# Tavish9/freegaussian

Hardware: AMD Instinct MI355X
Metric: Mpixels/s fwd+bwd @ 1M Gaussians 1080p (higher is better)
Workload: dtype f32; 1 GPU; north-star cfg4: 1000000 Gaussians, 1920x1080, SH degree 3, 1 view per rank per step, view = (rank + step) mod 8 around the 8-view ring, fwd+bwd, RGB, absgrad; layout=uniform, N=1000000, P=2073600, parallelism=view-dp1

## Files before the change

### freegaussian_amd/csrc/raster.hip

```cpp
#include "fg_common.h"

#include <stdlib.h>
#include <string.h>

#include <type_traits>

#include "jobs_build.h"

namespace {
using namespace fgjobs;

constexpr int TILE = 16;

__host__ __device__ constexpr int rec_vec4(int C) { return (6 + C + 3) / 4; }

__device__ __forceinline__ int tile_of_block(int b, int n, int tile_w, int tile_h, int mode) {
  const int xcd = b & 7, k = b >> 3;
  const int only = ((mode >> 8) & 15) - 1, kmod = mode >> 12;
  mode &= 255;
  if (only >= 0 && xcd != only) return -1;
  if (kmod > 1 && k % kmod != 0) return -1;
  if (mode == 0) {
    const int row = (k / tile_w) * 8 + xcd;
    return row < tile_h ? row * tile_w + (k % tile_w) : -1;
// ... 741 lines not shown
                                                     const int32_t* __restrict__ tile_offsets,
                                                     const int32_t* __restrict__ flatten_ids, float* __restrict__ render,
                                                     float* __restrict__ alphas, int32_t* __restrict__ last_ids,
                                                     const Composite& comp, float4* __restrict__ ckpt,
                                                     uint32_t* __restrict__ live_words,
                                                     const int32_t* __restrict__ slot_tab, long long* __restrict__ walk_out,
                                                     int seg_fine) {
  constexpr int C = 3, NV = rec_vec4(C);
  constexpr float MAY_STOP = FG_T_STOP * 1.00001f;
  const int tile_y = tile / tile_w, tile_x = tile - tile_y * tile_w;
  const int n_tiles = tile_w * ((height + TILE - 1) / TILE);
  const int start = tile_offsets[tile], end = tile_offsets[tile + 1];
  const int slot0 = ckpt ? seg_slot_base(slot_tab, start, tile) : -1;
  if (slot0 < 0 || end - start <= FG_WIDE_PREFIX) return;
  float4* const slots = ckpt + seg_slots_offset4(n_tiles, width, height);
  const int lane = fg::lane_id(), w = __builtin_amdgcn_readfirstlane(threadIdx.x >> 6);
  FwdShared<3, 64>& st = sh.stage[w];
  const uint64_t lt_mask = (lane == 0) ? 0ull : (~0ull >> (64 - lane));
  const int col = lane & 15, row = 4 * strip + (lane >> 4);
  const int ix = tile_x * TILE + col, iy = tile_y * TILE + row;
  const bool inside = ix < width && iy < height;
  const size_t pix = (size_t)min(iy, height - 1) * width + min(ix, width - 1);
  const float px = (float)ix + 0.5f;
  const StripBounds sb = strip_bounds((float)(tile_x * TILE), (float)(tile_y * TILE));
  const float pyb = (float)(tile_y * TILE + (lane >> 4)) + 0.5f;
  const float strip_off = (float)(4 * strip);
  const uint64_t full = __ballot(true);
  {
    const float4 v = slots[seg_slot_index(slot0, start, start) * FG_SEG_SLOT4 + row * TILE + col];
    if (!__any(v.x > 0.f)) return;
    if (w == 0) {
      sh.base[lane] = make_float4(fabsf(v.x), v.y, v.z, v.w);
      sh.base_last[lane] = last_ids[pix];
      sh.base_w[lane] = -1;
      sh.base_fin[lane] = !(v.x > 0.f);
    }
  }
  int cnt = 0;
  int ev_mine = 0, sc_mine = 0;
  uint32_t vlo = 0, vhi = 0;
  auto walk = [&](int batch, float& T, float (&acc)[C], int& last, uint64_t& done, auto bits) {
    for (int n0 = 0; n0 < cnt; n0 += 8) {
      if (done == full) break;
      const int n1 = min(n0 + 8, cnt);
      unsigned next_v = st.list[0][n0];
      for (int n = n0; n < n1; ++n) {
        const unsigned packed = __builtin_amdgcn_readfirstlane(next_v);
        next_v = st.list[0][min(n + 1, 63)];
        const int j = packed & 255u;
        Splat s;
        float f[C];
        read_record<C>(st.rec[j], s, f);
        const float dx = s.x - px, dy_base = s.y - pyb;
        const SigmaTerms sg = sigma_terms_prescaled(s.a, s.b, s.c, dx);
        const float dy = dy_base - strip_off;
        const float e2 = neg_sigma_log2e(sg, dy);
        const float alpha = fminf(FG_ALPHA_MAX, s.o * __builtin_amdgcn_exp2f(e2));
        const uint64_t valid = lanes_ule(e2, 0.f) & lanes_oge(alpha, FG_ALPHA_SKIP) & ~done;
        if (valid == 0ull) continue;
        if constexpr (decltype(bits)::value) {
          if (j < 32) vlo |= (uint32_t)lane_select(valid, 1 << j, 0);
          else vhi |= (uint32_t)lane_select(valid, 1 << (j - 32), 0);
        }
        const float next_T = T * (1.f - alpha);
        const uint64_t stop = valid & lanes_ole(next_T, FG_T_STOP);
        const uint64_t take = valid & ~stop;
        const float vis = lane_select0(take, alpha * T);
#pragma unroll
        for (int c = 0; c < C; ++c) acc[c] += f[c] * vis;
        last = lane_select(take, batch + j, last);
        T = lane_select(take, next_T, T);
        done |= stop;
      }
    }
  };

  float4 v_next[NV];
  {
    const int idx = start + FG_WIDE_PREFIX + 64 * w + lane;
    if (idx < end) {
      const float4* rec = splats + (size_t)flatten_ids[idx] * (FG_SPLAT_FLOATS / 4);
#pragma unroll
      for (int q = 0; q < NV; ++q) v_next[q] = rec[q];
    }
  }
  for (int r0 = start + FG_WIDE_PREFIX; r0 < end; r0 += 64 * NWV) {
    __syncthreads();
    const uint64_t done0 = __ballot(sh.base_fin[lane] != 0);
    if (done0 == full) break;
    const int batch = r0 + 64 * w;
    const int idx_next = batch + 64 * NWV + lane;
    const int gid_next = idx_next < end ? flatten_ids[idx_next] : 0;
    float T = 1.f, acc[C] = {0.f, 0.f, 0.f};
    int last = -1;
    uint64_t done = done0;
    cnt = 0;
    vlo = vhi = 0;
    if (batch < end) {
      const int idx = batch + lane;
      unsigned mask = 0;
      if (idx < end) {
        float4 v[NV];
#pragma unroll
        for (int q = 0; q < NV; ++q) v[q] = v_next[q];
        mask = strip_mask(v[0].x, v[0].y, v[0].z, v[0].w, v[1].x, v[1].y, sb);
        v[0].w *= 0.5f * FG_NEG_LOG2E;
        v[1].x *= FG_NEG_LOG2E;
        v[1].y *= 0.5f * FG_NEG_LOG2E;
#pragma unroll
        for (int q = 0; q < NV; ++q) st.rec[lane][q] = v[q];
      }
      const bool rel = (mask >> strip) & 1u;
      const uint64_t bal = __ballot(rel);
      if (rel) st.list[0][__popcll(bal & lt_mask)] = (uint16_t)(lane | (mask << 8));
      cnt = __popcll(bal);
      ev_mine += cnt;
      sc_mine += min(64, end - batch);
      __builtin_amdgcn_fence(__ATOMIC_RELEASE, "wavefront");
      __builtin_amdgcn_wave_barrier();
      __builtin_amdgcn_fence(__ATOMIC_ACQUIRE, "wavefront");
      walk(batch, T, acc, last, done, std::true_type{});
    }
    if (idx_next < end) {
      const float4* rec = splats + (size_t)gid_next * (FG_SPLAT_FLOATS / 4);
#pragma unroll
      for (int q = 0; q < NV; ++q) v_next[q] = rec[q];
    }
    {
      const bool stopped = ((done & ~done0) >> lane) & 1ull;
      sh.part[w][lane] = make_float4(stopped ? -1.f : T, acc[0], acc[1], acc[2]);
      sh.part_last[w][lane] = last;
    }
    if (lane < 2) sh.live_or[w][lane] = 0u;
    float t_in = 1.f, c_in[C] = {0.f, 0.f, 0.f};
    int l_in = start - 1, bw = -1;
    bool fin = false;
    float4 ck = make_float4(1.f, 0.f, 0.f, 0.f);
    float4 mp = make_float4(1.f, 0.f, 0.f, 0.f);
    __syncthreads();
    for (;;) {
      bw = sh.base_w[lane];
      fin = sh.base_fin[lane] != 0;
      l_in = sh.base_last[lane];
      {
        const float4 b = sh.base[lane];
        t_in = b.x; c_in[0] = b.y; c_in[1] = b.z; c_in[2] = b.w;
      }
      bool earlier = false;
      for (int q0 = 0; q0 < w; q0 += 5) {
        float4 pq[5];
        int plq[5];
#pragma unroll
        for (int u = 0; u < 5; ++u) {
          const int qq = min(q0 + u, NWV - 1);
          pq[u] = sh.part[qq][lane];
          plq[u] = sh.part_last[qq][lane];
        }
#pragma unroll
        for (int u = 0; u < 5; ++u) {
          const float4 p = pq[u];
          const int q = q0 + u;
          const bool use = q < w && q > bw && !fin && !earlier;
          const bool ms = use && (p.x < 0.f || t_in * p.x <= MAY_STOP);
          earlier = earlier || ms;
          if (use && !ms) {
            c_in[0] = fmaf(t_in, p.y, c_in[0]);
            c_in[1] = fmaf(t_in, p.z, c_in[1]);
            c_in[2] = fmaf(t_in, p.w, c_in[2]);
            t_in *= p.x;
            l_in = plq[u] >= 0 ? plq[u] : l_in;
          }
        }
      }
      mp = sh.part[w][lane];
      const bool reached = w > bw && !fin && !earlier;
      if (reached) ck = make_float4(t_in, c_in[0], c_in[1], c_in[2]);
      const bool mine = reached && (mp.x < 0.f || t_in * mp.x <= MAY_STOP);
      const uint64_t active = __ballot(mine);
      if (!__syncthreads_or(active != 0ull)) break;
      bool went_on = false;
      if (active != 0ull) {
        uint64_t d2 = ~active;
        walk(batch, t_in, c_in, l_in, d2, std::false_type{});
        if (mine) {
          sh.base[lane] = make_float4(t_in, c_in[0], c_in[1], c_in[2]);
          sh.base_last[lane] = l_in;
          sh.base_w[lane] = w;
          sh.base_fin[lane] = (int)((d2 >> lane) & 1ull);
          went_on = !((d2 >> lane) & 1ull);
        }
      }
      if (!__syncthreads_or(went_on)) {
        fin = sh.base_fin[lane] != 0;
        if (fin) l_in = sh.base_last[lane];
        if (fin) bw = sh.base_w[lane];
        break;
      }
    }
    if (batch > start && batch < end && seg_starts_at(batch - start, seg_fine))
      slots[seg_slot_index(slot0, start, batch, seg_fine) * FG_SEG_SLOT4 + row * TILE + col] = ck;
    if (live_words && batch < end) {
      const int rel_last = fin ? l_in - batch : 63;
      const uint32_t klo = rel_last < 0 ? 0u : (rel_last >= 31 ? ~0u : (2u << rel_last) - 1u);
      const uint32_t khi = rel_last < 32 ? 0u : (rel_last >= 63 ? ~0u : (2u << (rel_last - 32)) - 1u);
      if (vlo & klo) atomicOr(&sh.live_or[w][0], vlo & klo);
      if (vhi & khi) atomicOr(&sh.live_or[w][1], vhi & khi);
      __builtin_amdgcn_fence(__ATOMIC_RELEASE, "wavefront");
      __builtin_amdgcn_wave_barrier();
      __builtin_amdgcn_fence(__ATOMIC_ACQUIRE, "wavefront");
      const uint32_t word = sh.live_or[w][lane >> 5];
      if (batch + lane < end) reinterpret_cast<uint8_t*>(live_words + (batch + lane))[strip] = (uint8_t)((word >> (lane & 31)) & 1u);
    }
    if (w == NWV - 1) {
      if (!fin) {
        if (w > bw) {
          c_in[0] = fmaf(t_in, mp.y, c_in[0]);
          c_in[1] = fmaf(t_in, mp.z, c_in[1]);
          c_in[2] = fmaf(t_in, mp.w, c_in[2]);
          t_in *= mp.x;
          const int pl = sh.part_last[w][lane];
          l_in = pl >= 0 ? pl : l_in;
        }
        sh.base[lane] = make_float4(t_in, c_in[0], c_in[1], c_in[2]);
        sh.base_last[lane] = l_in;
      }
      sh.base_w[lane] = -1;
    }
  }
  __syncthreads();
  if (w != 0) return;
  const float4 b = sh.base[lane];
  const int last = sh.base_last[lane];
  float accf[C] = {b.y, b.z, b.w};
  {
    const int m = fg::wave_max_i32(last);
    if (lane == 0) reinterpret_cast<int32_t*>(ckpt)[4 * tile + strip] = m;
    const long long reach = (long long)(m - start + 1) * ev_mine / max(sc_mine, 1);
    if (walk_out && reach > FG_WALK_REPORT && lane == 0)
      __hip_atomic_store(walk_out, reach, __ATOMIC_RELAXED, __HIP_MEMORY_SCOPE_SYSTEM);
  }
  if (inside) {
    const float alpha_out = 1.f - b.x;
    reinterpret_cast<float*>(ckpt + seg_plane_offset4(n_tiles))[pix] = b.x;
    if (comp.background || comp.n_clamp > 0) {
      const float om = 1.f - alpha_out;
      unsigned blocked = 0;
#pragma unroll
      for (int c = 0; c < C; ++c) {
        float v = accf[c];
        if (comp.background) v += om * comp.background[c];
        if (c < comp.n_clamp) {
          if (v < 0.f || v > 1.f) blocked |= 1u << c;
          v = fminf(fmaxf(v, 0.f), 1.f);
        }
        accf[c] = v;
      }
      if (comp.n_clamp > 0) comp.clamp_mask[pix] = (uint8_t)blocked;
    }
#pragma unroll
    for (int c = 0; c < C; ++c) render[pix * C + c] = accf[c];
    alphas[pix] = alpha_out;
    last_ids[pix] = last;
  }
}

static_assert(sizeof(WideShared<FG_WIDE_WAVES>) <= 160 * 1024 / 2, "a wide job's stages: two workgroups per CU of gfx950's 160 KB LDS");
#if defined(__HIP_DEVICE_COMPILE__) && !defined(__gfx950__)
#error "libfgraster's kernels are written for gfx950 (MI355X): 160 KB of LDS per CU, wave64; build with --offload-arch=gfx950"
#endif
__global__ void __launch_bounds__(64 * FG_WIDE_WAVES)
raster_fwd_wide_kernel(int width, int height, int tile_w, int32_t* __restrict__ open_list,
                       const float4* __restrict__ splats, const int32_t* __restrict__ tile_offsets,
                       const int32_t* __restrict__ flatten_ids, float* __restrict__ render, float* __restrict__ alphas,
                       int32_t* __restrict__ last_ids, Composite comp, float4* __restrict__ ckpt,
                       uint32_t* __restrict__ live_words, const int32_t* __restrict__ slot_tab,
                       long long* __restrict__ walk_out, int seg_fine) {
  __shared__ WideShared<FG_WIDE_WAVES> sh;
  const int n_open = __builtin_amdgcn_readfirstlane(open_list[0]);
  for (int v = blockIdx.x; v < n_open; v += gridDim.x) {
    const int e = open_list[8 + v];
    FG_TL_BEGIN();
    raster_fwd_wide_body<FG_WIDE_WAVES>(sh, e >> 3, (e & 7) - 1, width, height, tile_w, splats, tile_offsets, flatten_ids,
                                        render, alphas, last_ids, comp, ckpt, live_words, slot_tab, walk_out, seg_fine);
    __syncthreads();
    FG_TL_END(1, e >> 3, (e & 7) - 1, 0, 3);
  }
  if (threadIdx.x == 0) {
    __threadfence();
    if (atomicAdd(&open_list[1], 1) == (int)gridDim.x - 1) {
      open_list[0] = 0;
      open_list[1] = 0;
    }
  }
}

template <int C, int NT>
struct BwdShared {
  float4 rec[NT][rec_vec4(C)];
  int32_t gid[NT];
  uint32_t mask[NT];
  alignas(16) float red[NT / 64][(8 + C) * fg::FG_RED_STRIDE];
  int32_t mx[NT / 64];
};

template <int C, int PPT, int NW, bool LIVE = false>
__device__ __forceinline__ void raster_bwd_body(BwdShared<C, 64 * NW>& sh, int tile, int wave_base, int width,
                                                int height, int tile_w, const float4* __restrict__ splats,
                                                const int32_t* __restrict__ tile_offsets,
                                                const int32_t* __restrict__ flatten_ids,
                                                const float* __restrict__ alphas,
                                                const int32_t* __restrict__ last_ids,
                                                const float* __restrict__ v_render,
                                                const float* __restrict__ v_alphas, float* __restrict__ v_splats,
                                                const Composite& comp, const Segments& seg = Segments{nullptr, nullptr, nullptr, 1, 0, 0},
                                                int part = 0, const uint32_t* __restrict__ live_words = nullptr) {
  constexpr int NT = 64 * NW;
  constexpr int RSTEP = TILE / PPT;
  constexpr int NV = rec_vec4(C);
  auto& lds = sh.rec;
  auto& lds_gid = sh.gid;
  auto& lds_mask = sh.mask;
  auto& lds_max = sh.mx;
  auto& lds_red = sh.red;
  const int tile_y = tile / tile_w, tile_x = tile - tile_y * tile_w;
  const int start = tile_offsets[tile], end = tile_offsets[tile + 1];
  if (end <= start) return;
  const int lane = fg::lane_id(), wl = NW == 1 ? 0 : __builtin_amdgcn_readfirstlane(threadIdx.x >> 6),
            wave = wave_base + wl;
  const int col = threadIdx.x & 15, row0 = 4 * wave_base + (threadIdx.x >> 4);
  const int ix = tile_x * TILE + col;
  const float px = (float)ix + 0.5f;
  const StripBounds sb = strip_bounds((float)(tile_x * TILE), (float)(tile_y * TILE));
  const unsigned my_strips = wave_strips<PPT>(wave);

  float T[PPT], rest[PPT], vr[PPT][C];
  const float pyb = (float)(tile_y * TILE + (int)(threadIdx.x >> 4) - 4 * wl) + 0.5f;
  int last[PPT];
  int my_max = start - 1;
  FG_TL_MARK(0);
  int lo = start, hi = end, bin_final = start - 1;
  int slot_last[PPT];
  bool from_ckpt = false;
  const float4* ck_slot = nullptr;
  bool share_job = false;
  if constexpr (C == 3 && NW == 1) share_job = seg.ckpt && seg.parts > 1;
  if (share_job) {
    const int4 tl = reinterpret_cast<const int4*>(seg.ckpt)[tile];
    const int tls[4] = {tl.x, tl.y, tl.z, tl.w};
#pragma unroll
    for (int k = 0; k < PPT; ++k) {
      slot_last[k] = __builtin_amdgcn_readfirstlane(tls[wave + k * (4 / PPT)]);
      bin_final = max(bin_final, slot_last[k]);
    }
    const int n_used = bin_final - start + 1;
    if (n_used <= 0) return;
    const int nseg = seg_count(n_used, seg.fine);
    const int c0 = part * nseg / seg.parts, c1 = (part + 1) * nseg / seg.parts;
    if (c0 == c1) return;
    lo = start + seg_bound(c0, seg.fine);
    hi = bin_final + 1;
    if (c1 < nseg) {
      hi = start + seg_bound(c1, seg.fine);
      from_ckpt = true;
      ck_slot = seg.ckpt + seg_slots_offset4(tile_w * ((height + TILE - 1) / TILE), width, height) +
                seg_slot_index(seg_slot_base(seg.slot_tab, start, tile), start, hi, seg.fine) * FG_SEG_SLOT4;
    }
  }
  FG_TL_MARK(1);
  struct Px {
    float alpha, va;
    int last;
    unsigned blocked;
    float v[C];
  } raw[PPT];
  float4 ckv[PPT];
  float cfv[PPT][3], tfe[PPT];
  const float* t_exact = nullptr;
  if constexpr (C == 3 && NW == 1) {
    if (from_ckpt)
      t_exact = reinterpret_cast<const float*>(seg.ckpt + seg_plane_offset4(tile_w * ((height + TILE - 1) / TILE)));
  }
  {
    const int ixc = min(ix, width - 1);
#pragma unroll
    for (int k = 0; k < PPT; ++k) {
      const int iyc = min(tile_y * TILE + row0 + k * RSTEP, height - 1);
      const size_t pix = (size_t)iyc * width + ixc;
      raw[k].alpha = alphas[pix];
      raw[k].last = last_ids[pix];
#pragma unroll
      for (int c = 0; c < C; ++c) raw[k].v[c] = v_render[pix * C + c];
    }
    if (v_alphas) {
#pragma unroll
      for (int k = 0; k < PPT; ++k)
        raw[k].va = v_alphas[(size_t)min(tile_y * TILE + row0 + k * RSTEP, height - 1) * width + ixc];
    } else {
#pragma unroll
      for (int k = 0; k < PPT; ++k) raw[k].va = 0.f;
    }
    if (comp.n_clamp > 0) {
#pragma unroll
      for (int k = 0; k < PPT; ++k)
        raw[k].blocked = comp.clamp_mask[(size_t)min(tile_y * TILE + row0 + k * RSTEP, height - 1) * width + ixc];
    } else {
#pragma unroll
      for (int k = 0; k < PPT; ++k) raw[k].blocked = 0u;
    }
#pragma unroll
    for (int k = 0; k < PPT; ++k) {
      ckv[k] = make_float4(1.f, 0.f, 0.f, 0.f);
      cfv[k][0] = cfv[k][1] = cfv[k][2] = 0.f;
      tfe[k] = 1.f;
    }
    if constexpr (C == 3 && NW == 1) {
      if (from_ckpt) {
#pragma unroll
        for (int k = 0; k < PPT; ++k) {
          const int iyc = min(tile_y * TILE + row0 + k * RSTEP, height - 1);
          const size_t pix = (size_t)iyc * width + ixc;
          ckv[k] = ck_slot[(row0 + k * RSTEP) * TILE + col];
          tfe[k] = t_exact[pix];
#pragma unroll
          for (int c = 0; c < 3; ++c) cfv[k][c] = seg.render_raw[pix * 3 + c];
        }
      }
    }
  }
#pragma unroll
  for (int k = 0; k < PPT; ++k) {
    const int iy = tile_y * TILE + row0 + k * RSTEP;
    const bool inside = ix < width && iy < height;
    const float alpha_f = inside ? raw[k].alpha : 0.f;
    T[k] = 1.f - alpha_f;
    last[k] = inside ? raw[k].last : start - 1;
    float va = inside ? raw[k].va : 0.f;
    const unsigned blocked = inside ? raw[k].blocked : 0u;
#pragma unroll
    for (int c = 0; c < C; ++c) {
      float v = inside ? raw[k].v[c] : 0.f;
      if ((blocked >> c) & 1u) v = 0.f;
      if (comp.background) va -= v * comp.background[c];
      vr[k][c] = v;
    }
    rest[k] = T[k] * va;
    if constexpr (C == 3 && NW == 1) {
      if (from_ckpt) {
        const float prefix[3] = {ckv[k].y, ckv[k].z, ckv[k].w};
        float sfx = 0.f;
#pragma unroll
        for (int c = 0; c < 3; ++c) {
          float f = cfv[k][c];
          if (comp.background) f -= (1.f - alpha_f) * comp.background[c];
          sfx += vr[k][c] * (f - prefix[c]);
        }
        const bool resume = last[k] >= hi;
        const float rho = T[k] * __builtin_amdgcn_rcpf(fmaxf(tfe[k], 1e-30f));
        T[k] = resume ? ckv[k].x * rho : T[k];
        rest[k] -= resume ? sfx * rho : 0.f;
      }
    }
    my_max = max(my_max, last[k]);
  }
  FG_TL_MARK(2);
  if (!share_job) {
    bin_final = __builtin_amdgcn_readfirstlane(fg::wave_max_i32(my_max));
    if (NW > 1) {
      if (lane == 0) lds_max[wl] = bin_final;
      __syncthreads();
#pragma unroll
      for (int w = 0; w < NW; ++w) bin_final = max(bin_final, lds_max[w]);
    }
    if (bin_final - start + 1 <= 0) return;
    hi = bin_final + 1;
    if constexpr (LIVE) {
#pragma unroll
      for (int k = 0; k < PPT; ++k) slot_last[k] = __builtin_amdgcn_readfirstlane(fg::wave_max_i32(last[k]));
    }
  }
  const int n_used = bin_final - start + 1;
  (void)n_used;
  const int n_batches = (hi - lo + NT - 1) / NT;
  if (threadIdx.x == 0) { FG_STAT(5, n_used); FG_STAT(6, end - start); }
  uint32_t red_wr[(8 + C + 3) / 4];
#pragma unroll
  for (int i = 0; i < (8 + C + 3) / 4; ++i) red_wr[i] = fg::lds_opaque(&lds_red[wl][4 * i * fg::FG_RED_STRIDE + lane]);
  float g[16];
#pragma unroll
  for (int q = 0; q < 16; ++q) asm volatile("v_mov_b32 %0, 0" : "=v"(g[q]));

  for (int b = n_batches - 1; b >= 0; --b) {
    const int batch = __builtin_amdgcn_readfirstlane(lo + b * NT);
    __syncthreads();
    FG_TL_STAGE_BEGIN();
    const int tl = NW == 1 ? fresh_lane_id() : (int)threadIdx.x;
    const int idx = batch + tl;
    unsigned mask = 0;
    const int gid_early = (LIVE && idx < hi) ? flatten_ids[idx] : 0;
    if constexpr (LIVE) {
      if (idx < hi) {
        const uint32_t lw = live_words[idx];
#pragma unroll
        for (int k = 0; k < PPT; ++k) {
          const int s4 = wave + k * (4 / PPT);
          if (((lw >> (8 * s4)) & 1u) && idx <= slot_last[k]) mask |= 1u << s4;
        }
      }
    }
    if (LIVE ? mask != 0u : idx < hi) {
      const int gid = LIVE ? gid_early : flatten_ids[idx];
      lds_gid[tl] = gid;
      const float4* rec = splats + (size_t)gid * (FG_SPLAT_FLOATS / 4);
      float4 v[NV];
#pragma unroll
      for (int q = 0; q < NV; ++q) v[q] = rec[q];
      if constexpr (!LIVE) mask = strip_mask(v[0].x, v[0].y, v[0].z, v[0].w, v[1].x, v[1].y, sb);
      if constexpr (C == 3) {
        v[2].y = v[0].w * (0.5f * FG_NEG_LOG2E);
        v[2].z = v[1].x * FG_NEG_LOG2E;
        v[2].w = v[1].y * (0.5f * FG_NEG_LOG2E);
      }
#pragma unroll
      for (int q = 0; q < NV; ++q) lds[tl][q] = v[q];
    }
    lds_mask[tl] = mask;
    __syncthreads();
    FG_TL_STAGE_END();
    for (int i = NT / 64 - 1; i >= 0; --i) {
      uint64_t todo = __ballot((lds_mask[64 * i + lane] & my_strips) != 0u);
      while (todo != 0ull) {
        const int bit = 63 - __builtin_clzll(todo);
        todo &= ~(1ull << bit);
        const int j = 64 * i + bit;
        const int idx_j = batch + j;
        if (NW > 1) {
          bool reach = false;
#pragma unroll
          for (int k = 0; k < PPT; ++k) reach = reach || (idx_j <= last[k]);
          if (!__any(reach)) continue;
        }

        FG_STAT(0, 1);
        Splat s;
        float f[C];
        read_record<C>(lds[j], s, f);
        const int gid_v = lds_gid[j];
        const float dx = s.x - px, dy_base = s.y - pyb;
        SigmaTerms st;
        if constexpr (C == 3) {
          const float4 tail = lds[j][2];
          st = sigma_terms_prescaled(tail.y, tail.z, tail.w, dx);
        } else {
          st = sigma_terms(s, dx);
        }
#define FG_BWD_SLOT_UPDATE(K, VALID, VIS, ALPHA)                                                        \
  do {                                                                                                  \
    FG_STAT(2, 1);                                                                                      \
    FG_STAT(3, __popcll(VALID));                                                                        \
    contributed = true;                                                                                 \
    const float dy = slot_dy<PPT>(dy_base, wave, K);                                                    \
    const float ov = s.o * (VIS);                                                                       \
    const float a_eff = lane_select0(VALID, ALPHA);                                                     \
    const float ra = __builtin_amdgcn_rcpf(1.f - a_eff);     \
    T[K] *= ra;                                                                                         \
    const float fac = a_eff * T[K];                                                                     \
    float cdot = 0.f;                                                                                   \
    _Pragma("unroll") for (int c = 0; c < C; ++c) {                                                     \
      g[8 + c] += fac * vr[K][c];                                                                       \
      cdot += f[c] * vr[K][c];                                                                          \
    }                                                                                                   \
     \
    const float v_alpha = fmaf(cdot, T[K], rest[K] * ra);                                               \
    rest[K] = fmaf(-cdot, fac, rest[K]);                                                                \
    const uint64_t open = (VALID) & lanes_ole(ov, FG_ALPHA_MAX);  \
    const float v_o = lane_select0(open, (VIS) * v_alpha);                             \
    const float v_sigma = -s.o * v_o;                                                                   \
    g[2] += v_o;                                                                                        \
                     \
    const float vsdy = v_sigma * dy;                                                                    \
    g[4] += vsdy;                                                                                       \
    g[5] = fmaf(vsdy, dy, g[5]);                                                                        \
        \
    g[6] = fmaf(fabsf(v_sigma), fabsf(fmaf(s.b, dy, adx)), g[6]);                                       \
    g[7] = fmaf(fabsf(v_sigma), fabsf(fmaf(s.c, dy, bdx)), g[7]);                                       \
  } while (0)
        bool contributed = false;
        const float adx = s.a * dx, bdx = s.b * dx;
        if constexpr (LIVE) {
          const unsigned smask = __builtin_amdgcn_readfirstlane(lds_mask[j]);
#pragma unroll
          for (int k = 0; k < PPT; ++k) {
            if (!((smask >> (wave + k * (4 / PPT))) & 1u)) continue;
            const float e2 = neg_sigma_log2e(st, slot_dy<PPT>(dy_base, wave, k));
            const float vis = __builtin_amdgcn_exp2f(e2);
            const float alpha = fminf(FG_ALPHA_MAX, s.o * vis);
            const uint64_t valid = lanes_sle(idx_j, last[k]) & lanes_ule(e2, 0.f) & lanes_uge(alpha, FG_ALPHA_SKIP);
            FG_STAT(1, 1);
            if (valid == 0ull) continue;
            FG_BWD_SLOT_UPDATE(k, valid, vis, alpha);
          }
        } else {
          float vis_k[PPT], alpha_k[PPT];
          uint64_t valid_k[PPT];
#pragma unroll
          for (int k = 0; k < PPT; ++k) {
            const float e2 = neg_sigma_log2e(st, slot_dy<PPT>(dy_base, wave, k));
            vis_k[k] = __builtin_amdgcn_exp2f(e2);
            alpha_k[k] = fminf(FG_ALPHA_MAX, s.o * vis_k[k]);
            valid_k[k] = lanes_sle(idx_j, last[k]) & lanes_ule(e2, 0.f) & lanes_uge(alpha_k[k], FG_ALPHA_SKIP);
            FG_STAT(1, 1);
          }
#pragma unroll
          for (int k = 0; k < PPT; ++k) {
            const uint64_t valid = valid_k[k];
            if (valid == 0ull) continue;
            FG_BWD_SLOT_UPDATE(k, valid, vis_k[k], alpha_k[k]);
          }
        }
#undef FG_BWD_SLOT_UPDATE
        if (!contributed) continue;
        {
          const float s0 = -s.o * g[2], s1 = g[4];
          g[0] = fmaf(s.b, s1, adx * s0);
          g[1] = fmaf(s.c, s1, bdx * s0);
          g[3] = (0.5f * dx * dx) * s0;
          g[4] = dx * s1;
          g[5] *= 0.5f;
        }
        FG_STAT(4, 1);
#if FG_BWD_LDS_REDUCE
        (void)lds_red;
        if (true) {
          const float total = fg::wave_reduce_rows_lds<8 + C>(g, red_wr, lds_red[wl], lane);
          if ((lane & 3) == 0 && (lane >> 2) < 8 + C) {
            const int gid_s = __builtin_amdgcn_readfirstlane(gid_v);
            float* dst = v_splats + (size_t)gid_s * FG_SPLAT_FLOATS + (lane >> 2);
            __hip_atomic_fetch_add(dst, total, __ATOMIC_RELAXED, __HIP_MEMORY_SCOPE_AGENT);
          }
        } else
#endif
        if (C <= 4) {
          const float total = fg::wave_reduce12_transposed(g);
          if (fg::wave_reduce12_owner(lane)) {
            const int gid_s = __builtin_amdgcn_readfirstlane(gid_v);
            float* dst = v_splats + (size_t)gid_s * FG_SPLAT_FLOATS + fg::wave_reduce12_index(lane);
            __hip_atomic_fetch_add(dst, total, __ATOMIC_RELAXED, __HIP_MEMORY_SCOPE_AGENT);
          }
        } else {
          const float total = fg::wave_reduce16_transposed(g);
          if ((lane & 3) == 0) {
            const int gid_s = __builtin_amdgcn_readfirstlane(gid_v);
            float* dst = v_splats + (size_t)gid_s * FG_SPLAT_FLOATS + (lane >> 2);
            __hip_atomic_fetch_add(dst, total, __ATOMIC_RELAXED, __HIP_MEMORY_SCOPE_AGENT);
          }
        }
        asm volatile("v_mov_b32 %0, 0" : "=v"(g[2]));
#pragma unroll
        for (int q = 4; q + 1 < 8 + C; q += 2) {
          struct F2 { float a, b; };
          double z;
          asm volatile("v_mov_b64 %0, 0" : "=v"(z));
          const F2 h = __builtin_bit_cast(F2, z);
          g[q] = h.a;
          g[q + 1] = h.b;
        }
        if ((8 + C) & 1) asm volatile("v_mov_b32 %0, 0" : "=v"(g[8 + C - 1]));
      }
    }
  }
}

template <int C, int PPT>
__global__ void __launch_bounds__(256 / PPT)
raster_bwd_kernel(int width, int height, int tile_w, int tile_h, int order_mode, const float4* __restrict__ splats,
                  const int32_t* __restrict__ tile_offsets, const int32_t* __restrict__ flatten_ids,
                  const float* __restrict__ alphas, const int32_t* __restrict__ last_ids,
                  const float* __restrict__ v_render, const float* __restrict__ v_alphas,
                  float* __restrict__ v_splats, Composite comp) {
  constexpr int NW = 256 / PPT / 64;
  __shared__ BwdShared<C, 64 * NW> sh;
  const int tile = tile_of_block(blockIdx.x, tile_w * tile_h, tile_w, tile_h, order_mode);
  if (tile < 0) return;
  raster_bwd_body<C, PPT, NW>(sh, tile, 0, width, height, tile_w, splats, tile_offsets, flatten_ids, alphas, last_ids,
                              v_render, v_alphas, v_splats, comp);
}

template <int C, bool LIVE>
__global__ void __launch_bounds__(64)
raster_bwd_mixed_kernel(int width, int height, int tile_w, int tile_h, int nx, int tail_tiles,
                        const int32_t* __restrict__ jobs, int cap,
                        const float4* __restrict__ splats, const int32_t* __restrict__ tile_offsets,
                        const int32_t* __restrict__ flatten_ids, const float* __restrict__ alphas,
                        const int32_t* __restrict__ last_ids, const float* __restrict__ v_render,
                        const float* __restrict__ v_alphas, float* __restrict__ v_splats, Composite comp,
                        Segments seg, const uint32_t* __restrict__ live_words) {
  __shared__ BwdShared<C, 64> sh;
  int strip = -1, part = 0, tile;
  if (seg.parts > 1) {
    if (jobs) {
      tile = share_from_list(blockIdx.x, jobs, cap, part, seg.parts);
    } else {
      const int xcd = blockIdx.x & 7, k = blockIdx.x >> 3;
      const Band band = band_of_xcd(xcd, tile_w, tile_h, nx);
      const int n = band.nrows * band.ncols;
      const int tail = seg.tail > 0 ? min(seg.tail, n) : n, n_main = n - tail;
      int t = k;
      if (k >= n_main) {
        t = n_main + (k - n_main) / seg.parts;
        part = ((k - n_main) - (t - n_main) * seg.parts + t) % seg.parts;
      } else {
        seg.parts = 1;
      }
      tile = job_of_block((t << 3) | xcd, tile_w, tile_h, nx, 0, strip);
    }
  } else {
    tile = jobs ? job_from_list(blockIdx.x, jobs, cap, strip)
                : job_of_block(blockIdx.x, tile_w, tile_h, nx, tail_tiles, strip);
  }
  if (tile < 0) return;
  FG_TL_BEGIN();
  if (seg.prio > 0) {
    const int len = tile_offsets[tile + 1] - tile_offsets[tile];
    job_priority(tile_offsets, tile_w * tile_h, seg.parts > 1 ? len / seg.parts : len, strip < 0 ? 13 : (strip >= 4 ? 10 : 8), seg.prio);
  }
  if (strip < 0)
    raster_bwd_body<C, 4, 1, LIVE>(sh, tile, 0, width, height, tile_w, splats, tile_offsets, flatten_ids, alphas,
                                   last_ids, v_render, v_alphas, v_splats, comp, seg, part, live_words);
  else if (strip >= 4)
    raster_bwd_body<C, 2, 1, LIVE>(sh, tile, strip - 4, width, height, tile_w, splats, tile_offsets, flatten_ids,
                                   alphas, last_ids, v_render, v_alphas, v_splats, comp, seg, part, live_words);
  else
    raster_bwd_body<C, 1, 1, LIVE>(sh, tile, strip, width, height, tile_w, splats, tile_offsets, flatten_ids, alphas,
                                   last_ids, v_render, v_alphas, v_splats, comp, seg, part, live_words);
  FG_TL_END(2, tile, strip, part, seg.parts);
}

__global__ void __launch_bounds__(256)
pack_splats_kernel(int N, int C, const float* __restrict__ means2d, const float* __restrict__ conics,
                   const float* __restrict__ opacities, const float* __restrict__ features,
                   float* __restrict__ splats) {
  const int64_t t = (int64_t)blockIdx.x * blockDim.x + threadIdx.x;
  const int64_t i = t >> 4;
  const int l = (int)(t & 15);
  if (i >= N) return;
  float v = 0.f;
  if (l < 2) v = means2d[2 * i + l];
  else if (l == 2) v = opacities[i];
  else if (l < 6) v = conics[3 * i + (l - 3)];
  else if (l - 6 < C) v = features[(size_t)i * C + (l - 6)];
  splats[i * FG_SPLAT_FLOATS + l] = v;
}

__global__ void __launch_bounds__(256)
unpack_grads_kernel(int N, int C, const float* __restrict__ v_splats, float* __restrict__ v_means2d,
                    float* __restrict__ v_means2d_abs, float* __restrict__ v_conics,
                    float* __restrict__ v_opacities, float* __restrict__ v_features) {
  const int64_t t = (int64_t)blockIdx.x * blockDim.x + threadIdx.x;
  const int64_t i = t >> 4;
  const int l = (int)(t & 15);
  if (i >= N) return;
  const float v = v_splats[i * FG_SPLAT_FLOATS + l];
  if (l < 2) {
    if (v_means2d) v_means2d[2 * i + l] = v;
  } else if (l == 2) {
    if (v_opacities) v_opacities[i] = v;
  } else if (l < 6) {
    if (v_conics) v_conics[3 * i + (l - 3)] = v;
  } else if (l < 8) {
    if (v_means2d_abs) v_means2d_abs[2 * i + (l - 6)] = v;
  } else if (l - 8 < C) {
    if (v_features) v_features[(size_t)i * C + (l - 8)] = v;
  }
}

using Cfg = fg_raster_config;
Cfg resolve(const fg_raster_config* c) {
  Cfg r;
  fg_raster_config_init(&r);
  if (c) {
    const size_t n = (size_t)c->size < sizeof(Cfg) ? (size_t)c->size : sizeof(Cfg);
    if (n >= sizeof(int32_t)) memcpy(&r, c, n);
    r.size = (int32_t)sizeof(Cfg);
  }
  return r;
}
int forced_ppt(int v) { return (v == 1 || v == 2 || v == 4) ? v : 0; }
int tile_order_mode(const Cfg& c) {
  const int order = (c.tile_order >= 0 && c.tile_order <= 5) ? c.tile_order : 2;
  const int only = (c.debug_only_xcd >= 0 && c.debug_only_xcd <= 7) ? ((c.debug_only_xcd + 1) << 8) : 0;
  return order | only | ((c.debug_k_mod > 0 ? c.debug_k_mod : 0) << 12);
}
int launch_grid(int mode, int tile_w, int tile_h) {
  switch (mode) {
    case 1: return tile_w * tile_h;
    case 3: return 8 * 2 * ((tile_h + 15) / 16) * tile_w;
    case 4: return 8 * ((tile_w + 3) / 4) * ((tile_h + 1) / 2);
    case 5: return 8 * ((tile_w + 1) / 2) * ((tile_h + 3) / 4);
    default: return 8 * ((tile_h + 7) / 8) * tile_w;
  }
}
int raster_ppt_fwd(const Cfg& c, int n_tiles) {
  const int forced = forced_ppt(c.ppt_fwd);
  if (forced) return forced;
  return n_tiles >= 6000 ? 2 : 1;
}
int raster_ppt_bwd(const Cfg& c, int n_tiles) {
  const int forced = forced_ppt(c.ppt_bwd);
  if (forced) return forced;
  return n_tiles >= 6000 ? 4 : (n_tiles >= 3000 ? 2 : 1);
}

template <int C, int PPT>
int launch_fwd(const Cfg& cfg, int width, int height, const float* splats, const int32_t* tile_offsets,
               const int32_t* flatten_ids, float* render, float* alphas, int32_t* last_ids, Composite comp,
               hipStream_t s) {
  const int tile_w = (width + TILE - 1) / TILE, tile_h = (height + TILE - 1) / TILE;
  const int mode = tile_order_mode(cfg);
  const int grid = launch_grid(mode & 255, tile_w, tile_h);
  hipLaunchKernelGGL((raster_fwd_kernel<C, PPT>), dim3(grid), dim3(256 / PPT), 0, s, width, height, tile_w,
                     tile_h, mode, reinterpret_cast<const float4*>(splats), tile_offsets, flatten_ids, render,
                     alphas, last_ids, comp);
  return hipGetLastError() == hipSuccess ? FG_OK : FG_ERR_LAUNCH;
}

template <int C, int PPT>
int launch_bwd(const Cfg& cfg, int width, int height, const float* splats, const int32_t* tile_offsets,
               const int32_t* flatten_ids, const float* alphas, const int32_t* last_ids, const float* v_render,
               const float* v_alphas, float* v_splats, Composite comp, hipStream_t s) {
  const int tile_w = (width + TILE - 1) / TILE, tile_h = (height + TILE - 1) / TILE;
  const int mode = tile_order_mode(cfg);
  const int grid = launch_grid(mode & 255, tile_w, tile_h);
  hipLaunchKernelGGL((raster_bwd_kernel<C, PPT>), dim3(grid), dim3(256 / PPT), 0, s, width, height, tile_w,
                     tile_h, mode, reinterpret_cast<const float4*>(splats), tile_offsets, flatten_ids, alphas,
                     last_ids, v_render, v_alphas, v_splats, comp);
  return hipGetLastError() == hipSuccess ? FG_OK : FG_ERR_LAUNCH;
}

#ifndef FG_SPLIT4_FWD
#define FG_SPLIT4_FWD 20
#endif
#ifndef FG_SPLIT2_FWD
#define FG_SPLIT2_FWD 16
#endif
#ifndef FG_SPLIT4_BWD
#define FG_SPLIT4_BWD 20
#endif
#ifndef FG_SPLIT2_BWD
#define FG_SPLIT2_BWD 16
#endif
#ifndef FG_TAIL4_TILES_FWD
#define FG_TAIL4_TILES_FWD 510
#endif
#ifndef FG_TAIL2_TILES_FWD
#define FG_TAIL2_TILES_FWD 0
#endif
#ifndef FG_TAIL4_TILES_BWD
#define FG_TAIL4_TILES_BWD 0
#endif
#ifndef FG_TAIL2_TILES_BWD
#define FG_TAIL2_TILES_BWD 300
#endif
#ifndef FG_MIXED_MIN_TILES
#define FG_MIXED_MIN_TILES 200
#endif
int raster_tail(const Cfg& cfg, int req4, int req2, int n_tiles, int dflt4, int dflt2) {
  int t4, t2 = 0;
  if (req4 >= 0) {
    t4 = req4;
    if (req2 > 0) t2 = req2;
  } else {
    if (n_tiles < FG_MIXED_MIN_TILES || (tile_order_mode(cfg) & 255) != 2 || (tile_order_mode(cfg) >> 8) != 0) return 0;
    const int per_xcd = n_tiles / 8;
    if (n_tiles < 5000) {
      t4 = dflt4 > 0 ? 0xFFFF : 0;
      t2 = dflt4 > 0 ? 0 : (dflt2 < per_xcd * 3 / 10 ? dflt2 : per_xcd * 3 / 10);
    } else {
      t4 = dflt4 < per_xcd / 2 ? dflt4 : per_xcd / 2;
      t2 = dflt2 < per_xcd * 3 / 10 ? dflt2 : per_xcd * 3 / 10;
    }
  }
  t4 = t4 < 0 ? 0 : (t4 > 0xFFFF ? 0xFFFF : t4);
  t2 = t2 < 0 ? 0 : (t2 > 0x7FFF ? 0x7FFF : t2);
  return t4 | (t2 << 16);
}
int mixed_tail_fwd(const Cfg& c, int n_tiles) {
  if (forced_ppt(c.ppt_fwd)) return 0;
  return raster_tail(c, c.tail4_fwd, c.tail2_fwd, n_tiles, FG_TAIL4_TILES_FWD, FG_TAIL2_TILES_FWD);
}
int mixed_tail_bwd(const Cfg& c, int n_tiles) {
  if (forced_ppt(c.ppt_bwd)) return 0;
  return raster_tail(c, c.tail4_bwd, c.tail2_bwd, n_tiles, FG_TAIL4_TILES_BWD, FG_TAIL2_TILES_BWD);
}
int band_tiles_for(int tile_w, int tile_h, int nx) {
  int m = 0;
  for (int x = 0; x < 8; ++x) {
    const Band b = band_of_xcd(x, tile_w, tile_h, nx);
    m = b.ncols * b.nrows > m ? b.ncols * b.nrows : m;
  }
  return m;
}
int band_nx(const Cfg& c) {
  const int v = c.bands_nx;
  return (v == 1 || v == 2 || v == 4 || v == 8) ? v : 1;
}
int band_rows_limit(const Cfg& c, int tile_h) {
  const int equal = (tile_h + 7) / 8;
  if (band_nx(c) != 1 || c.balance_bands == 0 || c.balance_bands == 2) return 0;
  const int lim = equal + (equal + 1) / 2;
  return lim < tile_h ? lim : tile_h;
}
int band_tiles_max(const Cfg& c, int tile_w, int tile_h) {
  const int rows = band_rows_limit(c, tile_h);
  return rows > 0 ? rows * tile_w : band_tiles_for(tile_w, tile_h, band_nx(c));
}
int mixed_grid(const Cfg& c, int tile_w, int tile_h, int tail) {
  const int n_max = band_tiles_max(c, tile_w, tile_h);
  int t4 = tail & 0xFFFF, t2 = tail >> 16;
  t4 = t4 < n_max ? t4 : n_max;
  t2 = t2 < n_max - t4 ? t2 : n_max - t4;
  return 8 * (n_max + 3 * t4 + t2);
}
int jobs_cap(const Cfg& c, int tile_w, int tile_h) { return 8 * band_tiles_max(c, tile_w, tile_h); }
int listed_grid(const Cfg& c, int tile_w, int tile_h, int tail) {
  const int g = mixed_grid(c, tile_w, tile_h, tail) / 8;
  const int cap = jobs_cap(c, tile_w, tile_h);
  const int want = g + band_tiles_max(c, tile_w, tile_h) / 2;
  return 8 * (want < cap ? want : cap);
}
int raster_split(int req4, int req2, int dflt4, int dflt2) {
  int s4 = dflt4, s2 = dflt2;
  if (req4 >= 0) {
    s4 = req4;
    s2 = req2 > 0 ? req2 : 0;
  }
  s4 = s4 < 0 ? 0 : (s4 > 0x7FFF ? 0x7FFF : s4);
  s2 = s2 < 0 ? 0 : (s2 > 0x7FFF ? 0x7FFF : s2);
  return s4 | (s2 << 16);
}

int seg_parts2(const Cfg& c);
int seg_tail2(const Cfg& c);
int seg_grid(const Cfg& c, int tile_w, int tile_h, int parts, int tail, bool listed) {
  const int n_max = band_tiles_max(c, tile_w, tile_h);
  const int split = tail > 0 ? (tail < n_max ? tail : n_max) : n_max;
  int per_xcd = n_max - split + split * parts + (listed ? n_max / 2 : 0);
  if (listed && seg_parts2(c) > parts) per_xcd += (seg_tail2(c) < split ? seg_tail2(c) : split) * (seg_parts2(c) - parts);
  const int cap = jobs_cap(c, tile_w, tile_h);
  return 8 * (listed && per_xcd > cap ? cap : per_xcd);
}
bool heavy_wide(const Cfg& c) { return c.heavy_wide != 0; }
int heavy_len(const Cfg& c) {
  const int least = heavy_wide(c) ? FG_WIDE_PREFIX + 256 : FG_HEAVY_PREFIX + 512;
  return c.heavy_tiles > 0 ? (c.heavy_tiles < least ? least : c.heavy_tiles) : 0;
}
#ifndef FG_SEG_FINE_DEFAULT
#define FG_SEG_FINE_DEFAULT 640
#endif
int seg_fine(const Cfg& c) {
  if (c.seg_fine == 0 || (heavy_len(c) > 0 && !heavy_wide(c))) return FG_SEG_FINE_NEVER;
  const int v = c.seg_fine < 0 ? FG_SEG_FINE_DEFAULT : c.seg_fine;
  return (v + 63) / 64 * 64;
}
int seg_slots(const Cfg& c) { return c.seg_slots > 0 ? (c.seg_slots + 7) / 8 * 8 : 0; }
int jobs_cap(const Cfg& c, int tile_w, int tile_h);
int64_t slot_table_offset(const Cfg& c, int tile_w, int tile_h) {
  return 8 + 8 * (int64_t)jobs_cap(c, tile_w, tile_h) + (heavy_len(c) > 0 ? FG_LOCAL_WORDS + FG_HEAVY_WORDS : 0);
}
const int32_t* slot_table(const Cfg& c, const int32_t* jobs, int tile_w, int tile_h) {
  return jobs && seg_slots(c) > 0 ? jobs + slot_table_offset(c, tile_w, tile_h) : nullptr;
}
#ifndef FG_PRIO_FWD_DEFAULT
#define FG_PRIO_FWD_DEFAULT (250 | 350 << 16)
#endif
#ifndef FG_PRIO_BWD_DEFAULT
#define FG_PRIO_BWD_DEFAULT (120 | 160 << 16)
#endif
int job_prio(int v, int dflt) { return v < 0 ? dflt : v; }
const uint32_t* live_use(const Cfg& c, const uint32_t* live_words) { return c.use_liveness == 0 ? nullptr : live_words; }
int seg_tail(const Cfg& c, int n_tiles) {
  return c.seg_tail >= 0 ? c.seg_tail : (n_tiles < 5000 ? 0 : FG_SEG_TAIL_DEFAULT);
}
int seg_tail_fit(const Cfg& c, int tile_w, int tile_h, int parts, int tail) {
  const int n_max = band_tiles_max(c, tile_w, tile_h);
  if (tail <= 0 || tail > n_max) tail = n_max;
  const int room = jobs_cap(c, tile_w, tile_h) - n_max - n_max / 2;
  const int fit = parts > 1 ? room / (parts - 1) : n_max;
  return tail < fit ? tail : (fit > 1 ? fit : 1);
}
#ifndef FG_SEG_PARTS2_DEFAULT
#define FG_SEG_PARTS2_DEFAULT 0
#endif
// ... 382 lines not shown
```

Before: 2896 Mpix/s.

## Slim LDS footprint of one-wave RGB backward job by keeping gid/mask in registers

For the single-wavefront RGB backward kernel, the shared-memory struct is specialised to hold only two float4s per splat plus the reduction buffer. The gid, third colour channel and strip mask now stay in the loading lane's registers and are fetched with readlane or ballot instead of LDS, and the prescaled sigma terms are recomputed per use. The kernel also gets a waves-per-EU hint so more blocks fit per CU. The aim is higher occupancy for latency hiding, paid for with extra ALU work per splat and a tighter register budget that could cause spills.

```diff
diff --git a/freegaussian_amd/csrc/raster.hip b/freegaussian_amd/csrc/raster.hip
--- a/freegaussian_amd/csrc/raster.hip
+++ b/freegaussian_amd/csrc/raster.hip
@@ -1067,6 +1067,12 @@
   alignas(16) float red[NT / 64][(8 + C) * fg::FG_RED_STRIDE];
   int32_t mx[NT / 64];
 };
+template <>
+struct BwdShared<3, 64> {
+  float4 rec[64][2];
+  alignas(16) float red[1][(8 + 3) * fg::FG_RED_STRIDE];
+};
+static_assert(sizeof(BwdShared<3, 64>) <= 5120, "the one-wavefront backward job: 32 images in a CU's 160 KB of LDS");
 
 template <int C, int PPT, int NW, bool LIVE = false>
 __device__ __forceinline__ void raster_bwd_body(BwdShared<C, 64 * NW>& sh, int tile, int wave_base, int width,
@@ -1082,10 +1088,8 @@
   constexpr int NT = 64 * NW;
   constexpr int RSTEP = TILE / PPT;
   constexpr int NV = rec_vec4(C);
+  constexpr bool SLIM = C == 3 && NW == 1;
   auto& lds = sh.rec;
-  auto& lds_gid = sh.gid;
-  auto& lds_mask = sh.mask;
-  auto& lds_max = sh.mx;
   auto& lds_red = sh.red;
   const int tile_y = tile / tile_w, tile_x = tile - tile_y * tile_w;
   const int start = tile_offsets[tile], end = tile_offsets[tile + 1];
@@ -1230,11 +1234,11 @@
   FG_TL_MARK(2);
   if (!share_job) {
     bin_final = __builtin_amdgcn_readfirstlane(fg::wave_max_i32(my_max));
-    if (NW > 1) {
-      if (lane == 0) lds_max[wl] = bin_final;
+    if constexpr (NW > 1) {
+      if (lane == 0) sh.mx[wl] = bin_final;
       __syncthreads();
 #pragma unroll
-      for (int w = 0; w < NW; ++w) bin_final = max(bin_final, lds_max[w]);
+      for (int w = 0; w < NW; ++w) bin_final = max(bin_final, sh.mx[w]);
     }
     if (bin_final - start + 1 <= 0) return;
     hi = bin_final + 1;
@@ -1261,6 +1265,8 @@
     const int tl = NW == 1 ? fresh_lane_id() : (int)threadIdx.x;
     const int idx = batch + tl;
     unsigned mask = 0;
+    int gid_keep = 0;
+    float f2_keep = 0.f;
     const int gid_early = (LIVE && idx < hi) ? flatten_ids[idx] : 0;
     if constexpr (LIVE) {
       if (idx < hi) {
@@ -1274,25 +1280,48 @@
     }
     if (LIVE ? mask != 0u : idx < hi) {
       const int gid = LIVE ? gid_early : flatten_ids[idx];
-      lds_gid[tl] = gid;
+      if constexpr (SLIM) gid_keep = gid;
+      else sh.gid[tl] = gid;
       const float4* rec = splats + (size_t)gid * (FG_SPLAT_FLOATS / 4);
       float4 v[NV];
 #pragma unroll
       for (int q = 0; q < NV; ++q) v[q] = rec[q];
       if constexpr (!LIVE) mask = strip_mask(v[0].x, v[0].y, v[0].z, v[0].w, v[1].x, v[1].y, sb);
-      if constexpr (C == 3) {
-        v[2].y = v[0].w * (0.5f * FG_NEG_LOG2E);
-        v[2].z = v[1].x * FG_NEG_LOG2E;
-        v[2].w = v[1].y * (0.5f * FG_NEG_LOG2E);
-      }
-#pragma unroll
-      for (int q = 0; q < NV; ++q) lds[tl][q] = v[q];
-    }
-    lds_mask[tl] = mask;
+      if constexpr (SLIM) {
+        f2_keep = v[2].x;
+        lds[tl][0] = v[0];
+        lds[tl][1] = v[1];
+      } else {
+        if constexpr (C == 3) {
+          v[2].y = v[0].w * (0.5f * FG_NEG_LOG2E);
+          v[2].z = v[1].x * FG_NEG_LOG2E;
+          v[2].w = v[1].y * (0.5f * FG_NEG_LOG2E);
+        }
+#pragma unroll
+        for (int q = 0; q < NV; ++q) lds[tl][q] = v[q];
+      }
+    }
+    if constexpr (!SLIM) sh.mask[tl] = mask;
     __syncthreads();
     FG_TL_STAGE_END();
     for (int i = NT / 64 - 1; i >= 0; --i) {
-      uint64_t todo = __ballot((lds_mask[64 * i + lane] & my_strips) != 0u);
+      uint64_t todo;
+      uint64_t slot_live[PPT];
+      (void)slot_live;
+      if constexpr (SLIM) {
+        if constexpr (LIVE) {
+          todo = 0ull;
+#pragma unroll
+          for (int k = 0; k < PPT; ++k) {
+            slot_live[k] = __ballot(((mask >> (wave + k * (4 / PPT))) & 1u) != 0u);
+            todo |= slot_live[k];
+          }
+        } else {
+          todo = __ballot((mask & my_strips) != 0u);
+        }
+      } else {
+        todo = __ballot((sh.mask[64 * i + lane] & my_strips) != 0u);
+      }
       while (todo != 0ull) {
         const int bit = 63 - __builtin_clzll(todo);
         todo &= ~(1ull << bit);
@@ -1308,11 +1337,22 @@
         FG_STAT(0, 1);
         Splat s;
         float f[C];
-        read_record<C>(lds[j], s, f);
-        const int gid_v = lds_gid[j];
+        int gid_v;
+        if constexpr (SLIM) {
+          const float4 v0 = lds[j][0], v1 = lds[j][1];
+          s.x = v0.x; s.y = v0.y; s.o = v0.z; s.a = v0.w; s.b = v1.x; s.c = v1.y;
+          f[0] = v1.z; f[1] = v1.w;
+          f[2] = __builtin_bit_cast(float, __builtin_amdgcn_readlane(__builtin_bit_cast(int, f2_keep), bit));
+          gid_v = __builtin_amdgcn_readlane(gid_keep, bit);
+        } else {
+          read_record<C>(lds[j], s, f);
+          gid_v = sh.gid[j];
+        }
         const float dx = s.x - px, dy_base = s.y - pyb;
         SigmaTerms st;
-        if constexpr (C == 3) {
+        if constexpr (SLIM) {
+          st = sigma_terms_prescaled(s.a * (0.5f * FG_NEG_LOG2E), s.b * FG_NEG_LOG2E, s.c * (0.5f * FG_NEG_LOG2E), dx);
+        } else if constexpr (C == 3) {
           const float4 tail = lds[j][2];
           st = sigma_terms_prescaled(tail.y, tail.z, tail.w, dx);
         } else {
@@ -1352,10 +1392,15 @@
         bool contributed = false;
         const float adx = s.a * dx, bdx = s.b * dx;
         if constexpr (LIVE) {
-          const unsigned smask = __builtin_amdgcn_readfirstlane(lds_mask[j]);
+          unsigned smask = 0u;
+          if constexpr (!SLIM) smask = __builtin_amdgcn_readfirstlane(sh.mask[j]);
 #pragma unroll
           for (int k = 0; k < PPT; ++k) {
-            if (!((smask >> (wave + k * (4 / PPT))) & 1u)) continue;
+            if constexpr (SLIM) {
+              if (!((slot_live[k] >> bit) & 1ull)) continue;
+            } else {
+              if (!((smask >> (wave + k * (4 / PPT))) & 1u)) continue;
+            }
             const float e2 = neg_sigma_log2e(st, slot_dy<PPT>(dy_base, wave, k));
             const float vis = __builtin_amdgcn_exp2f(e2);
             const float alpha = fminf(FG_ALPHA_MAX, s.o * vis);
@@ -1451,7 +1496,7 @@
 }
 
 template <int C, bool LIVE>
-__global__ void __launch_bounds__(64)
+__global__ void __launch_bounds__(64) __attribute__((amdgpu_waves_per_eu(C == 3 ? 7 : 1)))
 raster_bwd_mixed_kernel(int width, int height, int tile_w, int tile_h, int nx, int tail_tiles,
                         const int32_t* __restrict__ jobs, int cap,
                         const float4* __restrict__ splats, const int32_t* __restrict__ tile_offsets,
```

Measured after the change: 2929 Mpix/s, median of 6. 1.1% higher.
